# f90/Wave-U-Net

Measured on AMD Instinct MI355X. Metric: waveform samples/sec fwd+bwd, M1 12-level Wave-U-Net @1/2/4/8 GPU, higher is better.
Workload: dtype f32

## Files before the change

### wave-u-net_amd/csrc/wun_kernels.hip

```cpp
#include "wun_device.h"

#include <cstdio>
#include <cstdlib>
#include <map>
#include <mutex>
#include <string>
#include <algorithm>
#include <vector>

namespace wun {

__device__ __forceinline__ f32x4 mfma16(float a, float b, f32x4 c) {
    return __builtin_amdgcn_mfma_f32_16x16x4f32(a, b, c, 0, 0, 0);
}

__host__ __device__ static inline int fit_pitch(int width, int mod32) {
    return width + (((mod32 - (width % 32)) % 32) + 32) % 32;
}

struct ProfSlot { std::string name; std::string tag; double flops; double bytes; hipEvent_t e0, e1, c0, c1; };
static std::vector<ProfSlot> g_prof;
static bool g_prof_on = false;
static bool g_prof_detail = false;
static std::mutex g_prof_mu;
// ... 55 lines not shown
    std::map<std::string, Agg> agg;
    std::string detail;
    std::vector<float> empty_ms;
    for (auto& sl : g_prof) {
        (void)hipEventSynchronize(sl.c1);
        float ms = 0.f, cms = 0.f;
        if (hipEventElapsedTime(&cms, sl.c0, sl.c1) == hipSuccess) empty_ms.push_back(cms);
        if (hipEventElapsedTime(&ms, sl.e0, sl.e1) == hipSuccess) {
            Agg& a = agg[sl.name]; a.n += 1; a.ms += ms; a.flops += sl.flops; a.bytes += sl.bytes;
            if (g_prof_detail) {
                char buf[512];
                snprintf(buf, sizeof(buf), "%s{\"name\": \"%s\", \"tag\": \"%s\", \"ms\": %.6f, \"flops\": %.6e}",
                         detail.empty() ? "" : ", ", sl.name.c_str(), sl.tag.c_str(), ms, sl.flops);
                detail += buf;
            }
        }
        (void)hipEventDestroy(sl.e0); (void)hipEventDestroy(sl.e1); (void)hipEventDestroy(sl.c0); (void)hipEventDestroy(sl.c1);
    }
    g_prof.clear();
    double overhead_ms = 0.0;
    if (!empty_ms.empty()) {
        std::sort(empty_ms.begin(), empty_ms.end());
        overhead_ms = empty_ms[empty_ms.size() / 2];
    }
    char obuf[96];
    snprintf(obuf, sizeof(obuf), "{\"bracket_overhead_ms\": %.6f, ", overhead_ms);
    std::string out = std::string(obuf) + "\"launches\": [" + detail + "], \"kernels\": [";
    bool first = true;
    for (auto& kv : agg) {
        char buf[512];
        snprintf(buf, sizeof(buf), "%s{\"name\": \"%s\", \"launches\": %ld, \"ms\": %.6f, \"flops\": %.6e, \"bytes\": %.6e}",
                 first ? "" : ", ", kv.first.c_str(), kv.second.n, kv.second.ms, kv.second.flops, kv.second.bytes);
        out += buf;
        first = false;
    }
    out += "]}";
    return out;
}

#define WUN_JMAX 15


__device__ __forceinline__ int fast_div(int n, int d, float inv) {
    int q = (int)(((float)n + 0.5f) * inv);
    const int r = n - q * d;
    q += (r >= d) ? 1 : 0;
    q -= (r < 0) ? 1 : 0;
    return q;
}

#define WUN_FOLD_XCAP(TT) (3 * (TT) + 32)

__device__ __forceinline__ void conv_copy1(const ConvArgs& a, int b, int n, int q, float v) {
    if (a.dec != nullptr) {
        float* row = a.dec + (long long)b * a.decbs + (long long)n * a.decpitch + a.dec_off;
        if (a.dec_exp) {
            const unsigned pos = (unsigned)(2 * q - a.dec_lo);
            if (pos < a.dec_len) row[pos] = v;
        } else if ((q & 1) == 0) {
            row[q >> 1] = v;
        }
    }
    if (a.dec1 != nullptr && (q & 1) != 0) a.dec1[(long long)b * a.dec1bs + (long long)n * a.dec1pitch + a.dec1_off + (q >> 1)] = v;
}
__device__ __forceinline__ void conv_copy4(const ConvArgs& a, int b, int n, int q, f32x4 v) {
    if (a.dec != nullptr) {
        float* row = a.dec + (long long)b * a.decbs + (long long)n * a.decpitch + a.dec_off;
        if (a.dec_exp) {
            const int pos0 = 2 * q - a.dec_lo;
#pragma unroll
            for (int r = 0; r < 4; ++r)
                if ((unsigned)(pos0 + 2 * r) < a.dec_len) row[pos0 + 2 * r] = v[r];
        } else {
            row[q >> 1] = v[0];
            row[(q >> 1) + 1] = v[2];
        }
    }
    if (a.dec1 != nullptr) {
        float* row = a.dec1 + (long long)b * a.dec1bs + (long long)n * a.dec1pitch + a.dec1_off;
        row[q >> 1] = v[1];
        row[(q >> 1) + 1] = v[3];
    }
}
template <int MT, int NW, int WT, int WN, int CK, bool VECW, bool FOLD = false, bool XVEC = false, int KG = 1>
__global__ __launch_bounds__(256 * KG) void conv_mfma_kernel(ConvArgs a, int nTT, int nNT, int J,
                                                             int XP, int WP) {
    extern __shared__ __attribute__((aligned(16))) float lds_all[];
    const int kg = KG > 1 ? __builtin_amdgcn_readfirstlane((int)(threadIdx.x >> 8)) : 0;
    constexpr int TT = WT * MT * 16;
    constexpr int NT = WN * NW * 16;
    constexpr int NT4 = NT / 4;
    constexpr int CH = CK / 2;
    constexpr int TPR = 256 / CK;
    constexpr int XIT_D = FOLD ? (WUN_FOLD_XCAP(TT) + TPR - 1) / TPR : (TT + WUN_JMAX - 1 + TPR - 1) / TPR;
    constexpr int TPC = 256 / CH;
    constexpr int XIT_I = FOLD ? (2 * WUN_FOLD_XCAP(TT) + TPC - 1) / TPC
                               : (2 * (TT + (WUN_JMAX + 1) / 2 - 1) + TPC - 1) / TPC;
    constexpr int XIT = XVEC ? 1 : (XIT_D > XIT_I ? XIT_D : XIT_I);
    constexpr int WIT = XVEC ? 1 : (WUN_JMAX * CK * NT4 + 255) / 256;
    constexpr int XDIT = XVEC ? (CK * ((TT + 48) / 4) + 255) / 256 : 1;
    constexpr int WDIT = XVEC ? (WUN_JMAX * CK * (NT4 + 4) + 255) / 256 : 1;
    static_assert(!(XVEC && FOLD), "DMA staging is not implemented for batch-folded tiles");

    const int XB = CK * XP, LB = CK * XP + J * CK * WP;
    float* lds = lds_all + (KG > 1 ? kg * 2 * LB : 0);
    float* Xs = lds;
    float* Ws = lds + XB;

    const int tid = KG > 1 ? (int)(threadIdx.x & 255) : (int)threadIdx.x;
    const int lane = tid & 63;
    const int li = lane & 15, lg = lane >> 4;
    const int wave = __builtin_amdgcn_readfirstlane(tid >> 6);
#define WUN_PRIO_HI() __builtin_amdgcn_s_setprio(2)
#define WUN_PRIO_LO() __builtin_amdgcn_s_setprio(0)
    WUN_PRIO_HI();
    int bid = xcd_contiguous_block((int)blockIdx.x, (int)gridDim.x);
    const int nt = bid % nNT; bid /= nNT;
    const int tt = bid % nTT; bid /= nTT;
    const float inv_tout = 1.0f / (float)a.Tout;
    const int b = FOLD ? fast_div(tt * TT, a.Tout, inv_tout) : bid % a.B;
    const int ksg = FOLD ? bid : bid / a.B;
    const int ksp = ksg * KG + kg;
    const int q0 = tt * TT, n0 = nt * NT;
    int fold_nb = 1;
    const int fold_seg = a.Tout + J - 1;
    if constexpr (FOLD) {
        int last = fast_div(q0 + TT - 1, a.Tout, inv_tout);
        if (last > a.B - 1) last = a.B - 1;
        fold_nb = last - b + 1;
    }
    const int wt0 = (wave % WT) * MT * 16;
    const int wn0 = (wave / WT) * NW * 16;
    const int Ctot = a.C0 + a.C1;
    const bool deint = (a.loader == LOADER_DEINT);
    const bool phase2 = (a.flags & F_PHASE2) != 0;
    const int n0h = nt * (NT / 2);
    const int UW = FOLD ? fold_nb * fold_seg : TT + J - 1;
    const int CKC = deint ? CH : CK;
    const int nchunks = (Ctot + CKC - 1) / CKC;
    const int ch_lo = ksp * a.cps;
    int ch_hi = ch_lo + a.cps;
    if (ch_hi > nchunks) ch_hi = nchunks;

    const float* src0b = a.src0 + (long long)b * a.bs0 + a.off0;
    const float* src1b = (a.src1 != nullptr) ? a.src1 + (long long)b * a.bs1 + a.off1 : src0b;

    f32x4 acc[MT][NW];
#pragma unroll
    for (int m = 0; m < MT; ++m)
#pragma unroll
        for (int n = 0; n < NW; ++n) acc[m][n] = (f32x4){0.f, 0.f, 0.f, 0.f};

    float xreg[XIT];
    f32x4 wreg[WIT];
    unsigned xmask = 0, wmask = 0;

    int xt[XIT];
    unsigned xmask_s = 0, wmask_s = 0;
    const int xrow = deint ? tid / TPC : tid / TPR;
    const int dl0 = XVEC ? (((a.off0 - a.shift) % 4) + 4) % 4 : 0;
    const int dl1 = (XVEC && a.C1 > 0) ? (((a.off1 - a.shift) % 4) + 4) % 4 : dl0;
    int xdo[XDIT], wdo[WDIT];
    int nvr = 1, e00 = 0, e01 = 0;
    bool xedge = false;
    const float* vb0 = a.src0 + (long long)b * a.bs0;
    const float* vb1 = (a.src1 != nullptr) ? a.src1 + (long long)b * a.bs1 : vb0;
    const int XG = XP >> 2, WG4 = WP >> 2;
    if constexpr (XVEC) {
        const int tbase = q0 - a.shift;
        nvr = (UW + (dl0 > dl1 ? dl0 : dl1) + 3) >> 2;
        e00 = a.off0 + tbase - dl0;
        e01 = a.off1 + tbase - dl1;
        const int tf0 = tbase - dl0, tf1 = tbase - dl1;
        xedge = tf0 < 0 || tf0 + 4 * nvr > a.Tin || (a.C1 > 0 && (tf1 < 0 || tf1 + 4 * nvr > a.Tin));
        const float inv_xg = 1.0f / (float)XG;
#pragma unroll
        for (int i = 0; i < XDIT; ++i) {
            const int f = tid + i * 256;
            const int row = fast_div(f, XG, inv_xg), g = f - row * XG;
            xdo[i] = (row < CK && g < nvr) ? (row << 20) | (4 * g) : -1;
        }
        const float inv_wg = 1.0f / (float)WG4;
#pragma unroll
        for (int i = 0; i < WDIT; ++i) {
            const int f = tid + i * 256;
            const int row = fast_div(f, WG4, inv_wg), c4 = f - row * WG4;
            const int j = row / CK, r = row - j * CK;
            const bool ok = j < J && c4 < NT4;
            int wo;
            if (!phase2) {
                int col = n0 + c4 * 4;
                col = col > a.N - 4 ? a.N - 4 : col;
                wo = (j * Ctot + r) * a.N + col;
            } else {
                const int x = c4 * 4, ph = x / (NT / 2), cl = x % (NT / 2);
                int col = n0h + cl;
                col = col > a.N - 4 ? a.N - 4 : col;
                wo = (j * Ctot + r) * (2 * a.N) + ph * a.N + col;
            }
            wdo[i] = ok ? wo : -1;
        }
    }
    if constexpr (!XVEC) {
        const int lr = deint ? tid % TPC : tid % TPR;
        const int stride_i = deint ? TPC : TPR;
        const int lim = deint ? 2 * UW : UW;
        const int tbase = (deint ? 2 * q0 : q0) - a.shift;
        const int seglen = deint ? 2 * fold_seg : fold_seg;
        const float inv_seglen = 1.0f / (float)seglen;
#pragma unroll
        for (int i = 0; i < XIT; ++i) {
            const int u = lr + i * stride_i;
            int t = tbase + u, bl = 0;
            if constexpr (FOLD) { bl = fast_div(u, seglen, inv_seglen); t = u - bl * seglen - a.shift; }
            const bool ok = u < lim && t >= 0 && t < a.Tin;
            int tc = t < 0 ? 0 : t;
            if (tc > a.Tin - 1) tc = a.Tin - 1;
            if constexpr (FOLD) {
                if (bl > fold_nb - 1) bl = fold_nb - 1;
                tc |= bl << 20;
            }
            xt[i] = tc;
            xmask_s |= (ok ? 1u : 0u) << i;
        }
    }
    int wofs[WIT];
    int wr[WIT];
    const int nwvec = J * CK * NT4;
#pragma unroll
    for (int i = 0; i < (XVEC ? 0 : WIT); ++i) {
        const int f = tid + i * 256;
        const int row = f / NT4, c4 = f % NT4;
        const int j = row / CK, r = row % CK;
        int k, cch;
        if (!deint) { k = j; cch = r; }
        else { k = 2 * j + r / CH; cch = r % CH; }
        bool ok;
        int wo;
        if (!phase2) {
            ok = f < nwvec && k < a.KW && n0 + c4 * 4 < a.N;
            wo = (k * Ctot + cch) * a.N + n0 + c4 * 4;
        } else {
            const int x = c4 * 4, ph = x / (NT / 2), cl = x % (NT / 2);
            ok = f < nwvec && k < a.KW && n0h + cl < a.N;
            wo = (k * Ctot + cch) * (2 * a.N) + ph * a.N + n0h + cl;
        }
        wofs[i] = ok ? wo : 0;
        wr[i] = cch;
        wmask_s |= (ok ? 1u : 0u) << i;
    }

    auto load_chunk = [&](int chunk) {
        const int c0 = chunk * CKC;
        if constexpr (XVEC) {
            return;
        } else {
            const int c = c0 + xrow;
            const bool cok = c < Ctot;
            const float* p = (!cok || c < a.C0) ? src0b + (long long)(cok ? c : 0) * a.pitch0
                                                : src1b + (long long)(c - a.C0) * a.pitch1;
            const int nx = deint ? XIT_I : XIT_D;
            const int bsel = (!cok || c < a.C0) ? (int)a.bs0 : (int)a.bs1;
#pragma unroll
            for (int i = 0; i < XIT; ++i)
                if (i < nx) {
                    if constexpr (FOLD) xreg[i] = p[(xt[i] >> 20) * bsel + (xt[i] & 0xFFFFF)];
                    else xreg[i] = p[xt[i]];
                }
            xmask = cok ? xmask_s : 0u;
        }
        const bool tail = c0 + CKC > Ctot;
        const float* wc = a.W + (long long)c0 * (phase2 ? 2 * a.N : a.N);
        wmask = wmask_s;
#pragma unroll
        for (int i = 0; i < WIT; ++i) {
            if (i * 256 < nwvec) {
                const bool cok = !tail || c0 + wr[i] < Ctot;
                const float* wp = cok ? wc + wofs[i] : a.W;
                if constexpr (VECW) {
                    wreg[i] = *reinterpret_cast<const f32x4*>(wp);
                } else {
                    const int f = tid + i * 256;
                    const int c4 = f % NT4;
#pragma unroll
                    for (int e = 0; e < 4; ++e) {
                        const bool eok = n0 + c4 * 4 + e < a.N;
                        wreg[i][e] = eok ? wp[e] : 0.f;
                    }
                }
                if (!cok) wmask &= ~(1u << i);
            }
        }
    };
    auto store_chunk = [&](int bufoff, int chunk) {
        if constexpr (XVEC) {
            (void)chunk;
            return;
        } else if (!deint) {
            const int lr = tid % TPR;
            float* xd = Xs + bufoff + xrow * XP + lr;
#pragma unroll
            for (int i = 0; i < XIT_D; ++i)
                if (lr + i * TPR < UW) xd[i * TPR] = ((xmask >> i) & 1u) ? xreg[i] : 0.f;
        } else {
            const int le = tid % TPC;
            float* xd = Xs + bufoff + ((le & 1) * CH + xrow) * XP + (le >> 1);
#pragma unroll
            for (int i = 0; i < XIT_I; ++i)
                if (le + i * TPC < 2 * UW) xd[i * (TPC / 2)] = ((xmask >> i) & 1u) ? xreg[i] : 0.f;
        }
#pragma unroll
        for (int i = 0; i < WIT; ++i) {
            if (i * 256 < nwvec) {
                const int f = tid + i * 256;
                const int row = f / NT4, c4 = f % NT4;
                if (f < nwvec)
                    *reinterpret_cast<f32x4*>(&Ws[bufoff + row * WP + c4 * 4]) =
                        ((wmask >> i) & 1u) ? wreg[i] : (f32x4){0.f, 0.f, 0.f, 0.f};
            }
        }
    };

    constexpr int KS = CK / 4;
    int arow[MT];
#pragma unroll
    for (int m = 0; m < MT; ++m) {
        arow[m] = 0;
        if constexpr (FOLD) {
            const int row = q0 + wt0 + m * 16 + li;
            int g = fast_div(row, a.Tout, inv_tout);
            const int q = row - g * a.Tout;
            g -= b;
            arow[m] = g < fold_nb ? g * fold_seg + q : 0;
        }
    }
    const bool skip_last_odd = deint && CK == 8 && (a.KW & 1);
    auto run_taps = [&](int bufoff, int j_begin, int j_end, int dlt) {
        if (j_end <= j_begin) return;
        const float* xa = Xs + bufoff + lg * XP + (FOLD ? 0 : wt0 + li) + j_begin + (deint ? (dlt >> 1) : dlt);
        const int x2off = 4 * XP + (deint ? (dlt & 1) : 0);
        (void)x2off;
        const float* wb = Ws + bufoff + (j_begin * CK + lg) * WP + wn0 + li;
        const int wstep = CK * WP;
        float a0[MT], b0[NW], a1[MT], b1[NW];
        auto ldop = [&](const float* x, const float* w, float (&av)[MT], float (&bv)[NW]) {
#pragma unroll
            for (int m = 0; m < MT; ++m) av[m] = FOLD ? x[arow[m]] : x[m * 16];
#pragma unroll
            for (int n = 0; n < NW; ++n) bv[n] = w[n * 16];
        };
        auto mm_first = [&](const float (&av)[MT], const float (&bv)[NW]) {
            acc[0][0] = mfma16(av[0], bv[0], acc[0][0]);
        };
        auto mm_rest = [&](const float (&av)[MT], const float (&bv)[NW]) {
#pragma unroll
            for (int m = 0; m < MT; ++m)
#pragma unroll
                for (int n = 0; n < NW; ++n)
                    if (m + n > 0) acc[m][n] = mfma16(av[m], bv[n], acc[m][n]);
        };
        auto pin = [&]() {
            __builtin_amdgcn_sched_group_barrier(0x008, 1, 0);
            __builtin_amdgcn_sched_group_barrier(0x100, MT + NW, 0);
            __builtin_amdgcn_sched_group_barrier(0x008, MT * NW - 1, 0);
        };
        ldop(xa, wb, a0, b0);
        if constexpr (KS == 2) {
            const int j_full = (skip_last_odd && j_end == J) ? j_end - 1 : j_end;
            for (int j = j_begin; j < j_full; ++j) {
                const bool more = j + 1 < j_end;
                mm_first(a0, b0);
                ldop(xa + x2off, wb + 4 * WP, a1, b1);
                mm_rest(a0, b0);
                pin();
                xa += more ? 1 : 0;
                wb += more ? wstep : 0;
                mm_first(a1, b1);
                ldop(xa, wb, a0, b0);
                mm_rest(a1, b1);
                pin();
            }
            if (j_full < j_end) {
                mm_first(a0, b0);
                mm_rest(a0, b0);
            }
        } else {
            const int npair = (j_end - j_begin) / 2;
            int j = j_begin;
            for (int it = 0; it < npair; ++it, j += 2) {
                const bool more2 = j + 2 < j_end;
                mm_first(a0, b0);
                ldop(xa + 1, wb + wstep, a1, b1);
                mm_rest(a0, b0);
                pin();
                xa += more2 ? 2 : 1;
                wb += more2 ? 2 * wstep : wstep;
                mm_first(a1, b1);
                ldop(xa, wb, a0, b0);
                mm_rest(a1, b1);
                pin();
            }
            if (j < j_end) {
                mm_first(a0, b0);
                mm_rest(a0, b0);
            }
        }
    };

    auto dma_chunk = [&](int chunk, int bufoff) __attribute__((always_inline)) {
        if constexpr (XVEC) {
            const int c0 = chunk * CKC;
            const bool s1 = c0 >= a.C0;
            const float* xb = s1 ? vb1 + (long long)(c0 - a.C0) * a.pitch1 : vb0 + (long long)c0 * a.pitch0;
            const int pitch = s1 ? a.pitch1 : a.pitch0, e0s = s1 ? e01 : e00;
            const int nxg = CK * XG;
#pragma unroll
            for (int i = 0; i < XDIT; ++i) {
                if (i * 256 + wave * 64 < nxg) {
                    const int pk = xdo[i];
                    int e = e0s + (pk & 0xFFFFF);
                    e = e < 0 ? 0 : (e > pitch - 4 ? pitch - 4 : e);
                    if (pk >= 0)
                        __builtin_amdgcn_global_load_lds((gbl_cvoid_t*)(xb + (pk >> 20) * pitch + e),
                                                         (lds_void_t*)(Xs + bufoff + (i * 256 + wave * 64) * 4), 16, 0, 0);
                }
            }
            const float* wc = a.W + (long long)c0 * (phase2 ? 2 * a.N : a.N);
            const int nwg = J * CK * WG4;
#pragma unroll
            for (int i = 0; i < WDIT; ++i) {
                if (i * 256 + wave * 64 < nwg) {
                    const int o = wdo[i];
                    if (o >= 0)
                        __builtin_amdgcn_global_load_lds((gbl_cvoid_t*)(wc + o),
                                                         (lds_void_t*)(Ws + bufoff + (i * 256 + wave * 64) * 4), 16, 0, 0);
                }
            }
        }
    };
    auto zero_fix = [&](int chunk, int bufoff) __attribute__((always_inline)) {
        if constexpr (XVEC) {
            const bool s1 = chunk * CKC >= a.C0;
            const int t00 = (s1 ? e01 - a.off1 : e00 - a.off0);
            const float inv_xg = 1.0f / (float)XG;
#pragma unroll
            for (int i = 0; i < XDIT; ++i) {
                const int f = tid + i * 256;
                const int row = fast_div(f, XG, inv_xg), g = f - row * XG;
                if (row < CK && g < nvr) {
                    const int t0 = t00 + 4 * g;
#pragma unroll
                    for (int k = 0; k < 4; ++k)
                        if (t0 + k < 0 || t0 + k >= a.Tin) Xs[bufoff + row * XP + 4 * g + k] = 0.f;
                }
            }
        }
    };

    if constexpr (XVEC) {
        if (ch_lo < ch_hi) dma_chunk(ch_lo, 0);
        for (int chunk = ch_lo; chunk < ch_hi; ++chunk) {
            const int cur = ((chunk - ch_lo) & 1) * LB;
            asm volatile("s_waitcnt vmcnt(0)" ::: "memory");
            __syncthreads();
            if (chunk == ch_lo) WUN_PRIO_LO();
            if (xedge) {
                zero_fix(chunk, cur);
                __syncthreads();
            }
            if (chunk + 1 < ch_hi) dma_chunk(chunk + 1, LB - cur);
            run_taps(cur, 0, J, (chunk * CKC < a.C0) ? dl0 : dl1);
        }
    } else {
    if (ch_lo < ch_hi) load_chunk(ch_lo);
    if (ch_lo < ch_hi) store_chunk(0, ch_lo);
    __syncthreads();
    WUN_PRIO_LO();
    const int half = (J * 2) / 4;
    for (int chunk = ch_lo; chunk < ch_hi; ++chunk) {
        const int cur = ((chunk - ch_lo) & 1) * LB;
        const bool has_next = chunk + 1 < ch_hi;
        WUN_PRIO_HI();
        if (has_next) load_chunk(chunk + 1);
        WUN_PRIO_LO();
        run_taps(cur, 0, half, 0);
        WUN_PRIO_HI();
        if (has_next) store_chunk(LB - cur, chunk + 1);
        WUN_PRIO_LO();
        run_taps(cur, half, J, 0);
        __syncthreads();
    }
    }
    WUN_PRIO_HI();

    if constexpr (KG > 1) {
        __syncthreads();
        float* red = lds_all;
        if (kg > 0) {
#pragma unroll
            for (int m = 0; m < MT; ++m)
#pragma unroll
                for (int n = 0; n < NW; ++n)
                    *reinterpret_cast<f32x4*>(&red[((((kg - 1) * MT + m) * NW + n) * 256 + tid) * 4]) = acc[m][n];
        }
        __syncthreads();
        if (kg > 0) return;
#pragma unroll
        for (int g = 1; g < KG; ++g)
#pragma unroll
            for (int m = 0; m < MT; ++m)
#pragma unroll
                for (int n = 0; n < NW; ++n)
                    acc[m][n] += *reinterpret_cast<const f32x4*>(&red[((((g - 1) * MT + m) * NW + n) * 256 + tid) * 4]);
    }

    if (a.part != nullptr) {
        const int TP = (a.Tout + 3) & ~3;
#pragma unroll
        for (int n = 0; n < NW; ++n) {
            const int ncol = n0 + wn0 + n * 16 + li;
            if (ncol >= a.N) continue;
            float* prow = a.part + (((long long)ksg * a.B + b) * a.N + ncol) * TP;
#pragma unroll
            for (int m = 0; m < MT; ++m) {
                const int q = q0 + wt0 + m * 16 + lg * 4;
                if constexpr (FOLD) {
                    int g = fast_div(q, a.Tout, inv_tout), qq = q - g * a.Tout;
#pragma unroll
                    for (int r = 0; r < 4; ++r) {
                        if (g < a.B) a.part[(((long long)ksg * a.B + g) * a.N + ncol) * TP + qq] = acc[m][n][r];
                        if (++qq == a.Tout) { qq = 0; ++g; }
                    }
                } else {
                    if (q < TP) *reinterpret_cast<f32x4*>(&prow[q]) = acc[m][n];
                }
            }
        }
        return;
    }

    const AccRange rng = {a.acc_lo, a.acc_len};
    if (phase2) {
        if constexpr (WN == 1 && ((NW % 2) == 0 || NW == 3)) {
            const bool vec2 = (a.flags & F_VEC4) != 0;
            const bool accum2 = (a.flags & F_ACCUM) != 0;
            auto store8 = [&](int ncol, int m, float (&v)[8]) {
                const long long rowbase = (long long)b * a.obs0 + (long long)ncol * a.opitch0 + a.ooff0;
                const int q = q0 + wt0 + m * 16 + lg * 4;
                const int t0 = 2 * q;
                if (vec2 && t0 + 7 < a.Tlim) {
                    f32x4 w[2] = {{v[0], v[1], v[2], v[3]}, {v[4], v[5], v[6], v[7]}};
                    conv_out_vec<8>(a.dst0, a.msk0, rowbase + t0, accum2, rng, a.ooff0 + t0, w, NoCopy());
                } else {
#pragma unroll
// ... 261 lines not shown
    const ConvVariant& cv = kConvVariants[v];
    if (!cv.fold || (a.flags & F_PHASE2)) return false;
    const int TT = cv.WT * cv.MT * 16;
    const int J = a.loader == LOADER_DEINT ? (a.KW + 1) / 2 : a.KW;
    long long nb = (TT - 1) / a.Tout + 2;
    if (nb > a.B) nb = a.B;
    if (nb * (a.Tout + J - 1) > WUN_FOLD_XCAP(TT)) return false;
    if (a.Tin >= (1 << 20)) return false;
    const long long span0 = a.bs0 * (long long)a.B, span1 = a.src1 ? a.bs1 * (long long)a.B : 0;
    return span0 < (1ll << 31) && span1 < (1ll << 31);
}

static inline int conv_J(const ConvArgs& a) { return a.loader == LOADER_DEINT ? (a.KW + 1) / 2 : a.KW; }

static int pick_nw(int N, const int* cands, int ncand) {
    int best = cands[0], bestpad = 1 << 30;
    for (int i = 0; i < ncand; ++i) {
        const int nt = cands[i] * 16;
        const int padded = ((N + nt - 1) / nt) * nt;
        if (padded < bestpad) { bestpad = padded; best = cands[i]; }
    }
    return best;
}

int conv_pick_variant(const ConvArgs& a) {
    const int Ctot = a.C0 + a.C1;
    if (Ctot <= 4) return a.Tout > 64 ? 13 : 14;
    if (a.Tout <= 96 && a.B > 1 && (a.N & 3) == 0) {
        const int c[2] = {3, 2};
        const int nw = pick_nw(a.N, c, 2);
        const int v = ((long long)a.B * a.Tout >= 1024 ? 36 : 34) + (nw == 3 ? 1 : 0);
        if (conv_fold_ok(a, v)) return v;
    }
    if (a.Tout <= 16) return 12;
    if (a.Tout <= 32) { const int c[2] = {3, 2}; return pick_nw(a.N, c, 2) == 3 ? 11 : 10; }
    if (a.Tout <= 64) { const int c[2] = {3, 2}; return pick_nw(a.N, c, 2) == 3 ? 9 : 8; }
    const int pad256 = ((a.Tout + 255) / 256) * 256, pad128 = ((a.Tout + 127) / 128) * 128;
    const int base = (pad128 < pad256) ? 4 : 0;
    const int c[4] = {3, 5, 4, 2};
    const int nw = pick_nw(a.N, c, 4);
    return base + (nw - 2);
}

int conv_pick_variant_phase2(const ConvArgs& a) {
    const int pad256 = ((a.Tout + 255) / 256) * 256, pad128 = ((a.Tout + 127) / 128) * 128;
    const bool t128 = pad128 < pad256;
    int best = 2, bestpad = 1 << 30;
    const int cands[4] = {6, 4, 3, 2};
    for (int i = 0; i < 4; ++i) {
        const int half = cands[i] * 8;
        const int padded = ((a.N + half - 1) / half) * half;
        if (padded < bestpad) { bestpad = padded; best = cands[i]; }
    }
    if (best == 3) return t128 ? 5 : 1;
    if (best == 6) return 15;
    if (best == 4) return t128 ? 6 : 2;
    return t128 ? 4 : 0;
}

long long conv_natural_wgs_phase2(const ConvArgs& a) {
    const int v = conv_pick_variant_phase2(a);
    const int TT = kConvVariants[v].WT * kConvVariants[v].MT * 16;
    const int half = kConvVariants[v].NW * 8;
    return (long long)((a.Tout + TT - 1) / TT) * ((a.N + half - 1) / half) * a.B;
}

static inline int conv_J(const ConvArgs& a);
void conv_output_setup(ConvArgs& a) {
    if (a.acc_len == 0) { a.acc_lo = 0; a.acc_len = 0x7FFFFFFFu; }
    bool vec = a.ostride == 1 && aligned16(a.dst0) && (a.obs0 & 3) == 0 && (a.opitch0 & 3) == 0 && (a.ooff0 & 3) == 0;
    if (a.dst1 != nullptr)
        vec = vec && aligned16(a.dst1) && (a.obs1 & 3) == 0 && (a.opitch1 & 3) == 0 && (a.ooff1 & 3) == 0;
    if (a.msk0 != nullptr) vec = vec && aligned16(a.msk0);
    if (a.msk1 != nullptr) vec = vec && aligned16(a.msk1);
    if (a.dec != nullptr) vec = vec && (a.decpitch & 1) == 0 && (a.decbs & 1) == 0;
    if (vec) a.flags |= F_VEC4;
}

static int conv_dma_pitch(int width) { return fit_pitch((width + 3) & ~3, 16); }
static bool conv_xvec_ok(const ConvArgs& a, int variant, const WunSwitches& sw) {
    const ConvVariant& cv = kConvVariants[variant];
    const int Ctot = a.C0 + a.C1;
    if (cv.fold || cv.CK != 8 || sw.no_dma) return false;
    if (a.loader != LOADER_DIRECT) return false;
    const int CKC = cv.CK;
    if ((Ctot % CKC) != 0 || (a.C0 % CKC) != 0 || (a.N & 3) != 0 || a.N < 4) return false;
    if (!aligned16(a.src0) || (a.bs0 & 3) != 0 || (a.pitch0 & 3) != 0 || a.pitch0 < 4) return false;
    if (a.src1 != nullptr && (!aligned16(a.src1) || (a.bs1 & 3) != 0 || (a.pitch1 & 3) != 0 || a.pitch1 < 4)) return false;
    if (a.off0 < 0 || a.off1 < 0 || !aligned16(a.W)) return false;
    if ((long long)cv.CK * a.pitch0 >= (1ll << 31) || (long long)cv.CK * a.pitch1 >= (1ll << 31)) return false;
    return true;
}

static void conv_geom(const ConvArgs& a, int variant, const WunSwitches& sw, int& TT, int& NT, int& J, int& XP, int& WP) {
    const ConvVariant& v = kConvVariants[variant];
    TT = v.WT * v.MT * 16;
    NT = v.WN * v.NW * 16;
    J = conv_J(a);
    XP = fit_pitch(v.fold ? WUN_FOLD_XCAP(TT) : TT + J - 1, 16);
    if (conv_xvec_ok(a, variant, sw)) XP = conv_dma_pitch(TT + J - 1 + 3);
    WP = fit_pitch(NT, 16);
}

static inline long long conv_mtiles(const ConvArgs& a, int variant, int TT, int& bfac) {
    if (kConvVariants[variant].fold) { bfac = 1; return ((long long)a.B * a.Tout + TT - 1) / TT; }
    bfac = a.B;
    return (a.Tout + TT - 1) / TT;
}

size_t conv_lds_bytes(const ConvArgs& a, int variant, const WunSwitches& sw) {
    if (is_k3(variant)) {
        const int bv = conv_tile_variant(variant);
        const size_t stage = WUN_KG * conv_lds_bytes(a, bv, sw);
        const size_t red = (size_t)(WUN_KG - 1) * kConvVariants[bv].MT * kConvVariants[bv].NW * 256 * 16;
        return stage > red ? stage : red;
    }
    if (variant >= WUN_FIRST_RETIRED_VARIANT) return (size_t)1 << 30;
    int TT, NT, J, XP, WP;
    conv_geom(a, variant, sw, TT, NT, J, XP, WP);
    const int CK = kConvVariants[variant].CK;
    return 2 * sizeof(float) * ((size_t)CK * XP + (size_t)J * CK * WP);
}

double conv_flops(const ConvArgs& a) {
    if (a.flags & F_PHASE2)
        return 2.0 * a.kw_full * (double)(a.C0 + a.C1) * a.N * (double)a.Tin * a.B;
    return 2.0 * a.KW * (double)(a.C0 + a.C1) * a.N * (double)a.Tout * a.B;
}

void conv_splitk(const ConvArgs& a, int variant, const WunSwitches& sw, long long part_cap_floats, int& ksplit, int& cps) {
    int TT, NT, J, XP, WP;
    conv_geom(a, variant, sw, TT, NT, J, XP, WP);
    const int CK = kConvVariants[variant].CK;
    const int CKC = a.loader == LOADER_DEINT ? CK / 2 : CK;
    const int nchunks = (a.C0 + a.C1 + CKC - 1) / CKC;
    int bfac;
    const long long natural = conv_mtiles(a, variant, TT, bfac) * ((a.N + NT - 1) / NT) * bfac;
    ksplit = 1; cps = nchunks;
    if (natural >= 512 || nchunks < 2 || part_cap_floats <= 0) return;
    long long want = (1024 + natural - 1) / natural;
    if (want > nchunks) want = nchunks;
    const long long per = (long long)a.B * a.N * ((a.Tout + 3) & ~3);
    if (want * per > part_cap_floats) want = part_cap_floats / per;
    if (want < 2) return;
    cps = (int)((nchunks + want - 1) / want);
    ksplit = (nchunks + cps - 1) / cps;
    if (ksplit < 2) { ksplit = 1; cps = nchunks; }
}

template <int MT, int NW, int WT, int WN, int CK, bool VECW, bool FOLD = false, bool XVEC = false, int KG = 1>
static hipError_t conv_launch_t(ConvArgs a, int variant, float* part, long long part_cap, hipStream_t s, const WunSwitches& sw) {
    int TT, NT, J, XP, WP;
    conv_geom(a, variant, sw, TT, NT, J, XP, WP);
    const bool phase2 = (a.flags & F_PHASE2) != 0;
    int bfac;
    const int nTT = (int)conv_mtiles(a, variant, TT, bfac);
    const int nNT = phase2 ? (a.N + NT / 2 - 1) / (NT / 2) : (a.N + NT - 1) / NT;
    size_t lds = conv_lds_bytes(a, variant, sw);
    if (KG > 1) {
        const size_t red = (size_t)(KG - 1) * MT * NW * 256 * 16;
        lds = KG * lds > red ? KG * lds : red;
        if (phase2 || lds > 160 * 1024) return hipErrorInvalidValue;
    }
    if (FOLD && !conv_fold_ok(a, variant)) return hipErrorInvalidValue;
    auto kern = conv_mfma_kernel<MT, NW, WT, WN, CK, VECW, FOLD, XVEC, KG>;
    static size_t lds_allowed = 64 * 1024;
    if (lds > lds_allowed) {
        hipError_t e = hipFuncSetAttribute((const void*)kern, hipFuncAttributeMaxDynamicSharedMemorySize, (int)lds);
        if (e != hipSuccess) return e;
        lds_allowed = lds;
    }
    const size_t lds_launch = lds;
    int ksplit, cps;
    conv_splitk(a, variant, sw, (part != nullptr && !phase2) ? part_cap : 0, ksplit, cps);
    if (a.force_ksplit > 0 && !phase2) {
        const int CKC = a.loader == LOADER_DEINT ? CK / 2 : CK;
        const int nchunks = (a.C0 + a.C1 + CKC - 1) / CKC;
        int want = a.force_ksplit > nchunks ? nchunks : a.force_ksplit;
        if (part == nullptr) want = 1;
        const long long per = (long long)a.B * a.N * ((a.Tout + 3) & ~3);
        if (want > 1 && (long long)want * per > part_cap) return hipErrorInvalidValue;
        cps = (nchunks + want - 1) / want;
        ksplit = (nchunks + cps - 1) / cps;
    }
    if (KG > 1) {
        const int CKC = a.loader == LOADER_DEINT ? CK / 2 : CK;
        const int nchunks = (a.C0 + a.C1) / CKC;
        const int want = (a.force_ksplit > 0 && part != nullptr) ? a.force_ksplit : 1;
        if ((a.C0 + a.C1) % CKC != 0 || nchunks % (KG * want) != 0) return hipErrorInvalidValue;
        const long long per = (long long)a.B * a.N * ((a.Tout + 3) & ~3);
        if (want > 1 && (long long)want * per > part_cap) return hipErrorInvalidValue;
        ksplit = want;
        cps = nchunks / (KG * want);
    }
    a.cps = cps;
    a.part = ksplit > 1 ? part : nullptr;
    const long long grid = (long long)nTT * nNT * bfac * ksplit;
    if (grid <= 0) return hipSuccess;
    char nm[64];
    snprintf(nm, sizeof(nm), "conv_mfma_kernel<%d, %d, %d, %d, %d, %s%s%s%s>", MT, NW, WT, WN, CK, VECW ? "true" : "false",
             FOLD ? ", fold" : "", XVEC ? ", dma" : "", KG > 1 ? ", k3" : "");
    {
        char tag[160];
        snprintf(tag, sizeof(tag), "C=%d N=%d T=%d K=%d ld=%d B=%d ks=%d ph2=%d acc=%d os=%d grid=%lld", a.C0 + a.C1, a.N,
                 a.Tout, a.KW, a.loader, a.B, ksplit, (a.flags & F_PHASE2) ? 1 : 0, (a.flags & F_ACCUM) ? 1 : 0,
                 a.ostride, grid);
        ProfScope ps(nm, conv_flops(a), s, tag);
        hipLaunchKernelGGL(kern, dim3((unsigned)grid), dim3(256 * KG), lds_launch, s, a, nTT, nNT, J, XP, WP);
    }
    hipError_t e = hipGetLastError();
    if (e != hipSuccess || ksplit == 1) return e;
    const long long total = (long long)a.B * a.N * (((a.Tout + 3) & ~3) >> 2);
    long long blocks = (total + 255) / 256;
    if (blocks > 4096) blocks = 4096;
    {
        const double elems = (double)a.B * a.N * a.Tout;
        double by = 4.0 * elems * (ksplit + 1 + (a.msk0 != nullptr ? 1 : 0) + ((a.flags & F_ACCUM) ? 1 : 0));
        if (a.ups_y != nullptr) by += 4.0 * (double)a.B * a.N * a.ups_tup;
        ProfScope ps("conv_splitk_epilogue_kernel", 0.0, s, "", by);
        hipLaunchKernelGGL(conv_splitk_epilogue_kernel, dim3((unsigned)blocks), dim3(256), 0, s, a, ksplit);
    }
    t_last_fused_ups = (a.ups_y != nullptr || a.ubw_dz != nullptr) ? 1 : 0;
    return hipGetLastError();
}

bool conv_choice_ok(const ConvArgs& a, long long part_cap, int v, int ks, const WunSwitches& sw) {
    const int nvar = (int)(sizeof(kConvVariants) / sizeof(kConvVariants[0]));
    if (is_k3(v)) {
        const int bv = conv_tile_variant(v);
        if (sw.no_k3 || (a.flags & F_PHASE2) || ks < 1 || !conv_choice_ok(a, part_cap, bv, 1, sw)) return false;
        const ConvVariant& cv = kConvVariants[bv];
        const int CKC = a.loader == LOADER_DEINT ? cv.CK / 2 : cv.CK;
        const int Ctot = a.C0 + a.C1;
        if (Ctot % CKC) return false;
        const int nchunks = Ctot / CKC;
        if (nchunks % (WUN_KG * ks) != 0) return false;
        if (conv_lds_bytes(a, v, sw) > 160 * 1024) return false;
        const int TT = cv.WT * cv.MT * 16, NT = cv.WN * cv.NW * 16;
        int bfac;
        const long long natural = conv_mtiles(a, bv, TT, bfac) * ((a.N + NT - 1) / NT) * bfac;
        if (natural * ks > 2048) return false;
        const long long per = (long long)a.B * a.N * ((a.Tout + 3) & ~3);
        return ks == 1 || (long long)ks * per <= part_cap;
    }
    if (v >= WUN_FIRST_RETIRED_VARIANT) return false;
    if (v < 0 || v >= nvar || ks < 1) return false;
    const int Ctot = a.C0 + a.C1;
    const bool phase2 = (a.flags & F_PHASE2) != 0;
    if ((a.N & 3) != 0) return false;
    const ConvVariant& cv = kConvVariants[v];
    if (Ctot <= 4 && cv.CK != 4) return false;
    if (Ctot > 4 && cv.CK == 4 && (a.loader == LOADER_DEINT || phase2 || v < 26)) return false;
    if (phase2 && !(cv.WN == 1 && ((cv.NW % 2) == 0 || cv.NW == 3))) return false;
    if (cv.fold && !conv_fold_ok(a, v)) return false;
    const int TT = cv.WT * cv.MT * 16;
    const int NT = phase2 ? cv.WN * cv.NW * 8 : cv.WN * cv.NW * 16;
    if (!cv.fold && TT > 16 && TT >= 2 * a.Tout) return false;
    if (cv.fold && (long long)TT >= 2ll * a.B * a.Tout) return false;
    const int padded = ((a.N + NT - 1) / NT) * NT;
    if (padded * 3 > a.N * 4 + 48) return false;
    if (conv_lds_bytes(a, v, sw) > 150 * 1024) return false;
    if (ks == 1) return true;
    const int CKC = a.loader == LOADER_DEINT ? cv.CK / 2 : cv.CK;
    const int nchunks = (Ctot + CKC - 1) / CKC;
    int bfac;
    const long long natural = conv_mtiles(a, v, TT, bfac) * ((a.N + NT - 1) / NT) * bfac;
    const long long per = (long long)a.B * a.N * ((a.Tout + 3) & ~3);
    return !(phase2 || ks > nchunks || natural * ks > 6144 || (long long)ks * per > part_cap);
}

int conv_list_candidates(const ConvArgs& a, long long part_cap, ConvChoice* out, int maxn, const WunSwitches& sw) {
    int n = 0;
    const int nvar = conv_num_variants();
    static const int ks_menu[] = {1, 2, 3, 4, 6, 8, 12, 16, 24, 32, 48};
    for (int v = 0; v < nvar && n < maxn; ++v)
        for (unsigned i = 0; i < sizeof(ks_menu) / sizeof(ks_menu[0]) && n < maxn; ++i) {
            if (!conv_choice_ok(a, part_cap, v, ks_menu[i], sw)) {
                if (is_k3(v) && ks_menu[i] < 8) continue;
                break;
            }
            out[n].variant = v; out[n].ksplit = ks_menu[i]; ++n;
        }
    return n;
}

static_assert(sizeof(kConvVariants) / sizeof(kConvVariants[0]) == WUN_FIRST_RETIRED_VARIANT, "the retired index range follows the tile table");
static int first_k3_variant() { return WUN_FIRST_RETIRED_VARIANT + WUN_NUM_RETIRED_VARIANTS; }
int conv_num_variants() { return first_k3_variant() + kNumK3; }


int conv_last_fused_ups() { return t_last_fused_ups; }

hipError_t launch_conv(const ConvArgs& a_in, float* part, long long part_cap, hipStream_t s, const WunSwitches& sw) {
    ConvArgs a = a_in;
    t_last_fused_ups = 0;
    if (a.ups_y != nullptr && (a.dst1 != nullptr || a.msk0 != nullptr || a.ostride != 1 || a.ooff0 != 0 ||
                               (a.flags & (F_ACCUM | F_PHASE2)) != 0 || a.N0 != a.N || !aligned16(a.ups_y)))
        return hipErrorInvalidValue;
    if (a.ubw_dz != nullptr && (a.dst1 == nullptr || a.msk1 != nullptr || a.ostride != 1 || a.bias != nullptr ||
                                (a.flags & (F_ACCUM | F_PHASE2 | F_LRELU)) != 0 || a.N0 >= a.N || a.ubw_x == nullptr))
        return hipErrorInvalidValue;
    conv_output_setup(a);
    if (conv_J(a) > WUN_JMAX) return hipErrorInvalidValue;
    if (a.KW <= 0) {
        const long long total = (long long)a.B * a.N * (((a.Tout + 3) & ~3) >> 2);
        if (total <= 0) return hipSuccess;
        long long blocks = (total + 255) / 256;
        if (blocks > 4096) blocks = 4096;
        hipLaunchKernelGGL(conv_splitk_epilogue_kernel, dim3((unsigned)blocks), dim3(256), 0, s, a, 0);
        return hipGetLastError();
    }
    const bool vecw = (a.N & 3) == 0 && aligned16(a.W);
    if ((a.flags & F_PHASE2) && !(a.ostride == 1 && a.dst1 == nullptr && vecw)) return hipErrorInvalidValue;
    int v = (a.flags & F_PHASE2) ? conv_pick_variant_phase2(a) : conv_pick_variant(a);
    if (a.force_variant > 0 && vecw) {
        v = a.force_variant - 1;
        if (!conv_choice_ok(a, part != nullptr ? part_cap : 0, v, a.force_ksplit > 0 ? a.force_ksplit : 1, sw)) return hipErrorInvalidValue;
    }
    if (is_k3(v)) {
        const int bv = conv_tile_variant(v);
        const bool xv3 = conv_xvec_ok(a, bv, sw);
#define WUN_K3(i, MT, NW, WT, WN) case i: \
        if (xv3) return conv_launch_t<MT, NW, WT, WN, 8, true, false, true, WUN_KG>(a, bv, part, part_cap, s, sw); \
        return conv_launch_t<MT, NW, WT, WN, 8, true, false, false, WUN_KG>(a, bv, part, part_cap, s, sw);
#define WUN_K3F(i, MT, NW, WT, WN) case i: return conv_launch_t<MT, NW, WT, WN, 8, true, true, false, WUN_KG>(a, bv, part, part_cap, s, sw);
        switch (bv) {
            WUN_K3(8, 1, 2, 4, 1) WUN_K3(9, 1, 3, 4, 1) WUN_K3(10, 1, 2, 2, 2) WUN_K3(11, 1, 3, 2, 2)
            WUN_K3(4, 2, 2, 4, 1) WUN_K3(5, 2, 3, 4, 1)
            WUN_K3F(34, 1, 2, 4, 1) WUN_K3F(35, 1, 3, 4, 1) WUN_K3F(36, 2, 2, 4, 1) WUN_K3F(37, 2, 3, 4, 1)
            WUN_K3F(40, 2, 2, 2, 2)
            default: return hipErrorInvalidValue;
        }
#undef WUN_K3
#undef WUN_K3F
    }
    if (v >= WUN_FIRST_RETIRED_VARIANT) return hipErrorInvalidValue;
    if (!vecw) {
        const int Ctot = a.C0 + a.C1;
        if (Ctot <= 4) v = a.Tout > 64 ? 13 : 14;
        else v = a.Tout <= 16 ? 12 : (a.Tout <= 64 ? 9 : 1);
        switch (v) {
            case 1: return conv_launch_t<4, 3, 4, 1, 8, false>(a, v, part, part_cap, s, sw);
            case 9: return conv_launch_t<1, 3, 4, 1, 8, false>(a, v, part, part_cap, s, sw);
            case 12: return conv_launch_t<1, 2, 1, 4, 8, false>(a, v, part, part_cap, s, sw);
            case 13: return conv_launch_t<4, 2, 4, 1, 4, false>(a, v, part, part_cap, s, sw);
            default: return conv_launch_t<1, 2, 4, 1, 4, false>(a, v, part, part_cap, s, sw);
        }
    }
    const bool xv = conv_xvec_ok(a, v, sw);
#define WUN_CV(i, MT, NW, WT, WN, CK) case i: \
        if (xv) return conv_launch_t<MT, NW, WT, WN, CK, true, false, true>(a, v, part, part_cap, s, sw); \
        return conv_launch_t<MT, NW, WT, WN, CK, true>(a, v, part, part_cap, s, sw);
#define WUN_CV4(i, MT, NW, WT, WN, CK) case i: return conv_launch_t<MT, NW, WT, WN, CK, true>(a, v, part, part_cap, s, sw);
    switch (v) {
        WUN_CV(0, 4, 2, 4, 1, 8) WUN_CV(1, 4, 3, 4, 1, 8) WUN_CV(2, 4, 4, 4, 1, 8) WUN_CV(3, 4, 5, 4, 1, 8)
        WUN_CV(4, 2, 2, 4, 1, 8) WUN_CV(5, 2, 3, 4, 1, 8) WUN_CV(6, 2, 4, 4, 1, 8) WUN_CV(7, 2, 5, 4, 1, 8)
        WUN_CV(8, 1, 2, 4, 1, 8) WUN_CV(9, 1, 3, 4, 1, 8)
        WUN_CV(10, 1, 2, 2, 2, 8) WUN_CV(11, 1, 3, 2, 2, 8)
        WUN_CV(12, 1, 2, 1, 4, 8)
        WUN_CV4(13, 4, 2, 4, 1, 4) WUN_CV4(14, 1, 2, 4, 1, 4)
        WUN_CV(15, 2, 6, 4, 1, 8) WUN_CV(16, 4, 6, 4, 1, 8)
        WUN_CV(17, 3, 2, 4, 1, 8) WUN_CV(18, 3, 3, 4, 1, 8) WUN_CV(19, 3, 4, 4, 1, 8) WUN_CV(20, 3, 5, 4, 1, 8)
        WUN_CV(21, 3, 6, 4, 1, 8)
        WUN_CV(22, 5, 2, 4, 1, 8) WUN_CV(23, 5, 3, 4, 1, 8)
        WUN_CV(24, 6, 2, 4, 1, 8) WUN_CV(25, 6, 3, 4, 1, 8)
        WUN_CV4(26, 4, 3, 4, 1, 4) WUN_CV4(27, 2, 3, 4, 1, 4) WUN_CV4(28, 3, 3, 4, 1, 4) WUN_CV4(29, 2, 2, 4, 1, 4)
        WUN_CV4(30, 3, 2, 4, 1, 4) WUN_CV4(31, 4, 5, 4, 1, 4) WUN_CV4(32, 3, 5, 4, 1, 4) WUN_CV4(33, 2, 5, 4, 1, 4)
#define WUN_CF(i, MT, NW, WT, WN, CK) case i: return conv_launch_t<MT, NW, WT, WN, CK, true, true>(a, v, part, part_cap, s, sw);
        WUN_CF(34, 1, 2, 4, 1, 8) WUN_CF(35, 1, 3, 4, 1, 8) WUN_CF(36, 2, 2, 4, 1, 8) WUN_CF(37, 2, 3, 4, 1, 8)
        WUN_CF(38, 2, 3, 2, 2, 8) WUN_CF(39, 4, 3, 2, 2, 8) WUN_CF(40, 2, 2, 2, 2, 8) WUN_CF(41, 4, 2, 2, 2, 8)
#undef WUN_CF
        default: return hipErrorInvalidValue;
    }
#undef WUN_CV
#undef WUN_CV4
}

#define WUN_WG_XIT 8

template <int MTW, int NW, bool ACC = false>
__global__ __launch_bounds__(256, 2) void wgrad_mfma_kernel(WgradArgs a, int nMG, int nNG, int TK,
                                                         int XP, int ZP, int nChMax, int ONESP,
                                                         int XW4) {
    extern __shared__ __attribute__((aligned(16))) float lds[];
    constexpr int MG = 4 * MTW * 16;
    constexpr int NG = NW * 16;
    constexpr int ZIT = (NG * 32 + 255) / 256;
    const bool deint = (a.loader == LOADER_DEINT);
    const int planes = deint ? 2 : 1;
    float* Xs = lds + ONESP;
    float* Zs = Xs + nChMax * planes * XP;

    const int tid = threadIdx.x;
    const int lane = tid & 63;
    const int li = lane & 15, lg = lane >> 4;
    const int wave = __builtin_amdgcn_readfirstlane(tid >> 6);
    int bid = xcd_contiguous_block((int)blockIdx.x, (int)gridDim.x);
    const int ng = bid % nNG; bid /= nNG;
    const int mg = bid % nMG;
    const int split = bid / nMG;

    const int Ctot = a.C0 + a.C1;
    const int Mtot = Ctot * a.KW;
    const int rlo = mg * MG;
    const int cLo = rlo / a.KW;
    int cHi = (rlo + MG - 1) / a.KW;
    if (cHi > Ctot - 1) cHi = Ctot - 1;
    const int nCh = cHi - cLo + 1;

    const int delta0 = ((a.off0 - a.shift) % 4 + 4) % 4;
    const int delta1 = ((a.off1 - a.shift) % 4 + 4) % 4;

    int rowoff[MTW];
    int nact = 0;
#pragma unroll
    for (int mt = 0; mt < MTW; ++mt) {
        const int rt = rlo + (wave * MTW + mt) * 16;
        if (rt <= Mtot) nact = mt + 1;
        const int r = rt + li;
        int off = 0;
        if (r < Mtot) {
            const int c = r / a.KW, k = r - c * a.KW;
            const int kd = k + (c < a.C0 ? delta0 : delta1);
            off = ONESP + (c - cLo) * planes * XP + (deint ? ((kd & 1) * XP + (kd >> 1)) : kd);
        }
        rowoff[mt] = off;
    }
    for (int i = tid; i < ONESP; i += 256) lds[i] = 1.f;

    f32x4 acc[MTW][NW];
#pragma unroll
    for (int m = 0; m < MTW; ++m)
#pragma unroll
// ... 452 lines not shown
```

Baseline: 33.00 million.

## Add direct-to-LDS DMA staging path for stride-2 deinterleaved convolutions

Adds an S2 template mode so that convolutions using the deinterleaving loader (stride-2 downsampling) can use the global_load_lds DMA staging path, which was previously restricted to the direct loader. The stride-2 input is staged as four channel rows of raw interleaved samples, and tap addressing in LDS uses a doubled stride with a per-row parity offset. Weights are staged per original kernel tap rather than per folded J. The aim is to replace the register-based deinterleave loader with asynchronous DMA, lowering VGPR pressure and load latency. In exchange it adds edge-case patching code for the odd rows, halves channels per chunk, and LDS reads become strided, which may cause bank conflicts.

```diff
diff --git a/wave-u-net_amd/csrc/wun_kernels.hip b/wave-u-net_amd/csrc/wun_kernels.hip
--- a/wave-u-net_amd/csrc/wun_kernels.hip
+++ b/wave-u-net_amd/csrc/wun_kernels.hip
@@ -161,7 +161,7 @@
         row[(q >> 1) + 1] = v[3];
     }
 }
-template <int MT, int NW, int WT, int WN, int CK, bool VECW, bool FOLD = false, bool XVEC = false, int KG = 1>
+template <int MT, int NW, int WT, int WN, int CK, bool VECW, bool FOLD = false, bool XVEC = false, int KG = 1, bool S2 = false>
 __global__ __launch_bounds__(256 * KG) void conv_mfma_kernel(ConvArgs a, int nTT, int nNT, int J,
                                                              int XP, int WP) {
     extern __shared__ __attribute__((aligned(16))) float lds_all[];
@@ -180,8 +180,11 @@
     constexpr int XDIT = XVEC ? (CK * ((TT + 48) / 4) + 255) / 256 : 1;
     constexpr int WDIT = XVEC ? (WUN_JMAX * CK * (NT4 + 4) + 255) / 256 : 1;
     static_assert(!(XVEC && FOLD), "DMA staging is not implemented for batch-folded tiles");
-
-    const int XB = CK * XP, LB = CK * XP + J * CK * WP;
+    static_assert(!S2 || (XVEC && CK == 8), "the stride-2 DMA image is four channel rows of an 8-row tile");
+    constexpr int CKR = S2 ? CK / 2 : CK;
+    const int JW = S2 ? a.KW : J;
+
+    const int XB = CKR * XP, LB = CKR * XP + JW * CKR * WP;
     float* lds = lds_all + (KG > 1 ? kg * 2 * LB : 0);
     float* Xs = lds;
     float* Ws = lds + XB;
@@ -211,7 +214,7 @@
     const int wt0 = (wave % WT) * MT * 16;
     const int wn0 = (wave / WT) * NW * 16;
     const int Ctot = a.C0 + a.C1;
-    const bool deint = (a.loader == LOADER_DEINT);
+    const bool deint = S2 || (a.loader == LOADER_DEINT);
     const bool phase2 = (a.flags & F_PHASE2) != 0;
     const int n0h = nt * (NT / 2);
     const int UW = FOLD ? fold_nb * fold_seg : TT + J - 1;
@@ -246,26 +249,26 @@
     const float* vb1 = (a.src1 != nullptr) ? a.src1 + (long long)b * a.bs1 : vb0;
     const int XG = XP >> 2, WG4 = WP >> 2;
     if constexpr (XVEC) {
-        const int tbase = q0 - a.shift;
-        nvr = (UW + (dl0 > dl1 ? dl0 : dl1) + 3) >> 2;
+        const int tbase = (S2 ? 2 * q0 : q0) - a.shift;
+        nvr = ((S2 ? 2 * TT + a.KW : UW) + (dl0 > dl1 ? dl0 : dl1) + 3) >> 2;
         e00 = a.off0 + tbase - dl0;
         e01 = a.off1 + tbase - dl1;
-        const int tf0 = tbase - dl0, tf1 = tbase - dl1;
-        xedge = tf0 < 0 || tf0 + 4 * nvr > a.Tin || (a.C1 > 0 && (tf1 < 0 || tf1 + 4 * nvr > a.Tin));
+        const int tf0 = tbase - dl0 - (S2 ? 1 : 0), tf1 = tbase - dl1 - (S2 ? 1 : 0);
+        xedge = tf0 < 0 || tf0 + 4 * nvr + (S2 ? 1 : 0) > a.Tin || (a.C1 > 0 && (tf1 < 0 || tf1 + 4 * nvr + (S2 ? 1 : 0) > a.Tin));
         const float inv_xg = 1.0f / (float)XG;
 #pragma unroll
         for (int i = 0; i < XDIT; ++i) {
             const int f = tid + i * 256;
             const int row = fast_div(f, XG, inv_xg), g = f - row * XG;
-            xdo[i] = (row < CK && g < nvr) ? (row << 20) | (4 * g) : -1;
+            xdo[i] = (row < CKR && g < nvr) ? (row << 20) | (4 * g) : -1;
         }
         const float inv_wg = 1.0f / (float)WG4;
 #pragma unroll
         for (int i = 0; i < WDIT; ++i) {
             const int f = tid + i * 256;
             const int row = fast_div(f, WG4, inv_wg), c4 = f - row * WG4;
-            const int j = row / CK, r = row - j * CK;
-            const bool ok = j < J && c4 < NT4;
+            const int j = row / CKR, r = row - j * CKR;
+            const bool ok = j < JW && c4 < NT4;
             int wo;
             if (!phase2) {
                 int col = n0 + c4 * 4;
@@ -416,15 +419,16 @@
     const bool skip_last_odd = deint && CK == 8 && (a.KW & 1);
     auto run_taps = [&](int bufoff, int j_begin, int j_end, int dlt) {
         if (j_end <= j_begin) return;
-        const float* xa = Xs + bufoff + lg * XP + (FOLD ? 0 : wt0 + li) + j_begin + (deint ? (dlt >> 1) : dlt);
+        const float* xa = S2 ? Xs + bufoff + lg * XP + (lg & 1) + 2 * (wt0 + li) + j_begin + dlt
+                             : Xs + bufoff + lg * XP + (FOLD ? 0 : wt0 + li) + j_begin + (deint ? (dlt >> 1) : dlt);
         const int x2off = 4 * XP + (deint ? (dlt & 1) : 0);
         (void)x2off;
-        const float* wb = Ws + bufoff + (j_begin * CK + lg) * WP + wn0 + li;
-        const int wstep = CK * WP;
+        const float* wb = Ws + bufoff + (j_begin * CKR + lg) * WP + wn0 + li;
+        const int wstep = CKR * WP;
         float a0[MT], b0[NW], a1[MT], b1[NW];
         auto ldop = [&](const float* x, const float* w, float (&av)[MT], float (&bv)[NW]) {
 #pragma unroll
-            for (int m = 0; m < MT; ++m) av[m] = FOLD ? x[arow[m]] : x[m * 16];
+            for (int m = 0; m < MT; ++m) av[m] = FOLD ? x[arow[m]] : x[m * (S2 ? 32 : 16)];
 #pragma unroll
             for (int n = 0; n < NW; ++n) bv[n] = w[n * 16];
         };
@@ -444,7 +448,7 @@
             __builtin_amdgcn_sched_group_barrier(0x008, MT * NW - 1, 0);
         };
         ldop(xa, wb, a0, b0);
-        if constexpr (KS == 2) {
+        if constexpr (KS == 2 && !S2) {
             const int j_full = (skip_last_odd && j_end == J) ? j_end - 1 : j_end;
             for (int j = j_begin; j < j_full; ++j) {
                 const bool more = j + 1 < j_end;
@@ -492,20 +496,21 @@
             const bool s1 = c0 >= a.C0;
             const float* xb = s1 ? vb1 + (long long)(c0 - a.C0) * a.pitch1 : vb0 + (long long)c0 * a.pitch0;
             const int pitch = s1 ? a.pitch1 : a.pitch0, e0s = s1 ? e01 : e00;
-            const int nxg = CK * XG;
+            const int nxg = CKR * XG;
 #pragma unroll
             for (int i = 0; i < XDIT; ++i) {
                 if (i * 256 + wave * 64 < nxg) {
                     const int pk = xdo[i];
                     int e = e0s + (pk & 0xFFFFF);
                     e = e < 0 ? 0 : (e > pitch - 4 ? pitch - 4 : e);
+                    if constexpr (S2) e -= (pk >> 20) & 1;
                     if (pk >= 0)
                         __builtin_amdgcn_global_load_lds((gbl_cvoid_t*)(xb + (pk >> 20) * pitch + e),
                                                          (lds_void_t*)(Xs + bufoff + (i * 256 + wave * 64) * 4), 16, 0, 0);
                 }
             }
             const float* wc = a.W + (long long)c0 * (phase2 ? 2 * a.N : a.N);
-            const int nwg = J * CK * WG4;
+            const int nwg = JW * CKR * WG4;
 #pragma unroll
             for (int i = 0; i < WDIT; ++i) {
                 if (i * 256 + wave * 64 < nwg) {
@@ -526,11 +531,19 @@
             for (int i = 0; i < XDIT; ++i) {
                 const int f = tid + i * 256;
                 const int row = fast_div(f, XG, inv_xg), g = f - row * XG;
-                if (row < CK && g < nvr) {
-                    const int t0 = t00 + 4 * g;
+                if (row < CKR && g < nvr) {
+                    const int t0 = t00 + 4 * g - (S2 ? (row & 1) : 0);
 #pragma unroll
                     for (int k = 0; k < 4; ++k)
                         if (t0 + k < 0 || t0 + k >= a.Tin) Xs[bufoff + row * XP + 4 * g + k] = 0.f;
+                    if constexpr (S2) {
+                        const int pitch = s1 ? a.pitch1 : a.pitch0, off = s1 ? a.off1 : a.off0;
+                        if ((row & 1) && t0 + 1 + off > pitch - 4 && t0 >= 0 && t0 < a.Tin) {
+                            const float* xr = s1 ? vb1 + (long long)(chunk * CKC - a.C0 + row) * a.pitch1
+                                                 : vb0 + (long long)(chunk * CKC + row) * a.pitch0;
+                            Xs[bufoff + row * XP + 4 * g] = xr[off + t0];
+                        }
+                    }
                 }
             }
         }
@@ -548,7 +561,7 @@
                 __syncthreads();
             }
             if (chunk + 1 < ch_hi) dma_chunk(chunk + 1, LB - cur);
-            run_taps(cur, 0, J, (chunk * CKC < a.C0) ? dl0 : dl1);
+            run_taps(cur, 0, JW, (chunk * CKC < a.C0) ? dl0 : dl1);
         }
     } else {
     if (ch_lo < ch_hi) load_chunk(ch_lo);
@@ -976,8 +989,9 @@
     const ConvVariant& cv = kConvVariants[variant];
     const int Ctot = a.C0 + a.C1;
     if (cv.fold || cv.CK != 8 || sw.no_dma) return false;
-    if (a.loader != LOADER_DIRECT) return false;
-    const int CKC = cv.CK;
+    const bool s2 = a.loader == LOADER_DEINT;
+    if (s2 && (a.flags & F_PHASE2)) return false;
+    const int CKC = s2 ? cv.CK / 2 : cv.CK;
     if ((Ctot % CKC) != 0 || (a.C0 % CKC) != 0 || (a.N & 3) != 0 || a.N < 4) return false;
     if (!aligned16(a.src0) || (a.bs0 & 3) != 0 || (a.pitch0 & 3) != 0 || a.pitch0 < 4) return false;
     if (a.src1 != nullptr && (!aligned16(a.src1) || (a.bs1 & 3) != 0 || (a.pitch1 & 3) != 0 || a.pitch1 < 4)) return false;
@@ -992,7 +1006,9 @@
     NT = v.WN * v.NW * 16;
     J = conv_J(a);
     XP = fit_pitch(v.fold ? WUN_FOLD_XCAP(TT) : TT + J - 1, 16);
-    if (conv_xvec_ok(a, variant, sw)) XP = conv_dma_pitch(TT + J - 1 + 3);
+    if (conv_xvec_ok(a, variant, sw)) {
+        XP = a.loader == LOADER_DEINT ? (2 * TT + a.KW - 1 + 3 + 1 + 3) & ~3 : conv_dma_pitch(TT + J - 1 + 3);
+    }
     WP = fit_pitch(NT, 16);
 }
 
@@ -1013,6 +1029,8 @@
     int TT, NT, J, XP, WP;
     conv_geom(a, variant, sw, TT, NT, J, XP, WP);
     const int CK = kConvVariants[variant].CK;
+    if (a.loader == LOADER_DEINT && conv_xvec_ok(a, variant, sw))
+        return 2 * sizeof(float) * ((size_t)(CK / 2) * XP + (size_t)a.KW * (CK / 2) * WP);
     return 2 * sizeof(float) * ((size_t)CK * XP + (size_t)J * CK * WP);
 }
 
@@ -1042,7 +1060,7 @@
     if (ksplit < 2) { ksplit = 1; cps = nchunks; }
 }
 
-template <int MT, int NW, int WT, int WN, int CK, bool VECW, bool FOLD = false, bool XVEC = false, int KG = 1>
+template <int MT, int NW, int WT, int WN, int CK, bool VECW, bool FOLD = false, bool XVEC = false, int KG = 1, bool S2 = false>
 static hipError_t conv_launch_t(ConvArgs a, int variant, float* part, long long part_cap, hipStream_t s, const WunSwitches& sw) {
     int TT, NT, J, XP, WP;
     conv_geom(a, variant, sw, TT, NT, J, XP, WP);
@@ -1057,7 +1075,7 @@
         if (phase2 || lds > 160 * 1024) return hipErrorInvalidValue;
     }
     if (FOLD && !conv_fold_ok(a, variant)) return hipErrorInvalidValue;
-    auto kern = conv_mfma_kernel<MT, NW, WT, WN, CK, VECW, FOLD, XVEC, KG>;
+    auto kern = conv_mfma_kernel<MT, NW, WT, WN, CK, VECW, FOLD, XVEC, KG, S2>;
     static size_t lds_allowed = 64 * 1024;
     if (lds > lds_allowed) {
         hipError_t e = hipFuncSetAttribute((const void*)kern, hipFuncAttributeMaxDynamicSharedMemorySize, (int)lds);
@@ -1093,7 +1111,7 @@
     if (grid <= 0) return hipSuccess;
     char nm[64];
     snprintf(nm, sizeof(nm), "conv_mfma_kernel<%d, %d, %d, %d, %d, %s%s%s%s>", MT, NW, WT, WN, CK, VECW ? "true" : "false",
-             FOLD ? ", fold" : "", XVEC ? ", dma" : "", KG > 1 ? ", k3" : "");
+             FOLD ? ", fold" : "", XVEC ? (S2 ? ", dma2" : ", dma") : "", KG > 1 ? ", k3" : "");
     {
         char tag[160];
         snprintf(tag, sizeof(tag), "C=%d N=%d T=%d K=%d ld=%d B=%d ks=%d ph2=%d acc=%d os=%d grid=%lld", a.C0 + a.C1, a.N,
@@ -1215,6 +1233,7 @@
         const int bv = conv_tile_variant(v);
         const bool xv3 = conv_xvec_ok(a, bv, sw);
 #define WUN_K3(i, MT, NW, WT, WN) case i: \
+        if (xv3 && a.loader == LOADER_DEINT) return conv_launch_t<MT, NW, WT, WN, 8, true, false, true, WUN_KG, true>(a, bv, part, part_cap, s, sw); \
         if (xv3) return conv_launch_t<MT, NW, WT, WN, 8, true, false, true, WUN_KG>(a, bv, part, part_cap, s, sw); \
         return conv_launch_t<MT, NW, WT, WN, 8, true, false, false, WUN_KG>(a, bv, part, part_cap, s, sw);
 #define WUN_K3F(i, MT, NW, WT, WN) case i: return conv_launch_t<MT, NW, WT, WN, 8, true, true, false, WUN_KG>(a, bv, part, part_cap, s, sw);
@@ -1243,6 +1262,7 @@
     }
     const bool xv = conv_xvec_ok(a, v, sw);
 #define WUN_CV(i, MT, NW, WT, WN, CK) case i: \
+        if (xv && a.loader == LOADER_DEINT) return conv_launch_t<MT, NW, WT, WN, CK, true, false, true, 1, true>(a, v, part, part_cap, s, sw); \
         if (xv) return conv_launch_t<MT, NW, WT, WN, CK, true, false, true>(a, v, part, part_cap, s, sw); \
         return conv_launch_t<MT, NW, WT, WN, CK, true>(a, v, part, part_cap, s, sw);
 #define WUN_CV4(i, MT, NW, WT, WN, CK) case i: return conv_launch_t<MT, NW, WT, WN, CK, true>(a, v, part, part_cap, s, sw);
```

After: 33.32 million (median of 6 runs). No clear change (+0.9%).
